# marcinmiklitz/pywindow

Measured on AMD Instinct MI355X. Metric: trajectory frames/sec full_analysis (pore+windows), CC3 1k-frame, higher is better.
Workload: dtype f64

## Files before the change

### pywindow_amd/csrc/pw_team.hpp

```cpp
#pragma once
#include "pw_common.hpp"

namespace pw {

struct HostTeam {
    static constexpr int NWAVES = 1;
    static constexpr int WSIZE = 1;
    static constexpr int SIZE = 1;
    PW_HD static int tid() { return 0; }
    PW_HD static int lane() { return 0; }
    PW_HD static int wave() { return 0; }
    PW_HD static void sync() {}
    PW_HD static void wave_sync() {}
    PW_HD static void wave_argmin(double& v, int& idx) { (void)v; (void)idx; }
    PW_HD static void wave_argmax(double& v, int& idx) { (void)v; (void)idx; }
    PW_HD static void row_argmin4(double v, int idx, double* outv, int* outi) {
        for (int r = 0; r < 4; ++r) { outv[r] = v; outi[r] = idx; }
    }
    PW_HD static double wave_min(double v) { return v; }
    PW_HD static void row_min4(double v, double* outv) { for (int r = 0; r < 4; ++r) outv[r] = v; }
    PW_HD static unsigned long long ballot(bool p) { return p ? 1ull : 0ull; }
    PW_HD static bool wave_all(bool p) { return p; }
    PW_HD static bool wave_any(bool p) { return p; }
    PW_HD static double xor_d(double v, int ) { return v; }
    PW_HD static double bcast(double v, int ) { return v; }
    PW_HD static double bcast_u(double v, int ) { return v; }
    PW_HD static int bcast_i(int v, int ) { return v; }
    PW_HD static int shfl_up_i(int v, int ) { return v; }
    PW_HD static int uniform_i(int v) { return v; }
};

#if defined(__HIPCC__)
#if defined(PW_BARRIER_PROF)
__shared__ unsigned long long pw_bar_acc[8];
#endif
template <int NW>
struct DeviceTeam {
    static constexpr int NWAVES = NW;
    static constexpr int WSIZE = 64;
    static constexpr int SIZE = NW * 64;
    __device__ static int tid() { return threadIdx.x; }
    __device__ static int lane() { return threadIdx.x & 63; }
    __device__ static int wave() { return threadIdx.x >> 6; }
#if defined(PW_BARRIER_PROF)
    __device__ static void sync() {
        const long long t0 = wall_clock64();
        __syncthreads();
        if (lane() == 0) atomicAdd(&pw_bar_acc[wave()], (unsigned long long)(wall_clock64() - t0));
    }
#else
    __device__ static void sync() { __syncthreads(); }
#endif
    __device__ static void wave_sync() {
        __builtin_amdgcn_fence(__ATOMIC_RELEASE, "wavefront");
#if defined(PW_GENERIC_TEAM_MEM)
        asm volatile("s_waitcnt vmcnt(0) lgkmcnt(0)" ::: "memory");
#endif
        __builtin_amdgcn_wave_barrier();
        __builtin_amdgcn_fence(__ATOMIC_ACQUIRE, "wavefront");
    }
    template <int CTRL, int ROW_MASK, int BANK_MASK>
    __device__ static int dpp_i(int x) {
        return __builtin_amdgcn_update_dpp(x, x, CTRL, ROW_MASK, BANK_MASK, false);
    }
    template <int CTRL, int ROW_MASK, int BANK_MASK>
    __device__ static double dpp_d(double x) {
        union { double d; int i[2]; } a, b;
        a.d = x;
        b.i[0] = dpp_i<CTRL, ROW_MASK, BANK_MASK>(a.i[0]);
        b.i[1] = dpp_i<CTRL, ROW_MASK, BANK_MASK>(a.i[1]);
        return b.d;
    }
    __device__ static double lane_d(double x, int lane) {
        union { double d; int i[2]; } a;
        a.d = x;
        a.i[0] = __builtin_amdgcn_readlane(a.i[0], lane);
        a.i[1] = __builtin_amdgcn_readlane(a.i[1], lane);
        return a.d;
    }
    template <bool IS_MIN, int CTRL, int ROW_MASK, int BANK_MASK>
    __device__ static void arg_step(double& v, int& idx) {
        double ov = dpp_d<CTRL, ROW_MASK, BANK_MASK>(v);
        int oi = dpp_i<CTRL, ROW_MASK, BANK_MASK>(idx);
        bool take = IS_MIN ? ((ov < v) || (ov == v && oi < idx)) : ((ov > v) || (ov == v && oi < idx));
        v = take ? ov : v;
        idx = take ? oi : idx;
    }
    template <bool IS_MIN>
    __device__ static void arg_reduce16(double& v, int& idx) {
        arg_step<IS_MIN, 0x111, 0xf, 0xf>(v, idx);
        arg_step<IS_MIN, 0x112, 0xf, 0xf>(v, idx);
        arg_step<IS_MIN, 0x114, 0xf, 0xe>(v, idx);
        arg_step<IS_MIN, 0x118, 0xf, 0xc>(v, idx);
    }
    template <bool IS_MIN>
    __device__ static void arg_reduce64(double& v, int& idx) {
        arg_reduce16<IS_MIN>(v, idx);
        arg_step<IS_MIN, 0x142, 0xa, 0xf>(v, idx);
        arg_step<IS_MIN, 0x143, 0xc, 0xf>(v, idx);
        v = lane_d(v, 63);
        idx = __builtin_amdgcn_readlane(idx, 63);
    }
    __device__ static void wave_argmin(double& v, int& idx) { arg_reduce64<true>(v, idx); }
    __device__ static void wave_argmax(double& v, int& idx) { arg_reduce64<false>(v, idx); }
    __device__ static void row_argmin4(double v, int idx, double* outv, int* outi) {
        arg_reduce16<true>(v, idx);
        outv[0] = lane_d(v, 15); outi[0] = __builtin_amdgcn_readlane(idx, 15);
        outv[1] = lane_d(v, 31); outi[1] = __builtin_amdgcn_readlane(idx, 31);
        outv[2] = lane_d(v, 47); outi[2] = __builtin_amdgcn_readlane(idx, 47);
        outv[3] = lane_d(v, 63); outi[3] = __builtin_amdgcn_readlane(idx, 63);
    }
    template <int CTRL, int ROW_MASK, int BANK_MASK>
    __device__ static void min_step(double& v) {
        v = __builtin_fmin(v, dpp_d<CTRL, ROW_MASK, BANK_MASK>(v));
    }
    __device__ static double wave_min(double v) {
        min_step<0x111, 0xf, 0xf>(v);
        min_step<0x112, 0xf, 0xf>(v);
        min_step<0x114, 0xf, 0xe>(v);
        min_step<0x118, 0xf, 0xc>(v);
        min_step<0x142, 0xa, 0xf>(v);
        min_step<0x143, 0xc, 0xf>(v);
        return lane_d(v, 63);
    }
    __device__ static void row_min4(double v, double* outv) {
        min_step<0x111, 0xf, 0xf>(v);
        min_step<0x112, 0xf, 0xf>(v);
        min_step<0x114, 0xf, 0xe>(v);
        min_step<0x118, 0xf, 0xc>(v);
        outv[0] = lane_d(v, 15); outv[1] = lane_d(v, 31); outv[2] = lane_d(v, 47); outv[3] = lane_d(v, 63);
    }
    __device__ static unsigned long long ballot(bool p) { return __ballot(p); }
    __device__ static bool wave_all(bool p) { return __all(p); }
    __device__ static bool wave_any(bool p) { return __any(p); }
    __device__ static double xor_d(double v, int lane_mask) { return __shfl_xor(v, lane_mask, 64); }
    __device__ static double bcast(double v, int src) { return __shfl(v, src, 64); }
    __device__ static double bcast_u(double v, int src) { return lane_d(v, __builtin_amdgcn_readfirstlane(src)); }
    __device__ static int bcast_i(int v, int src) { return __shfl(v, src, 64); }
    __device__ static int shfl_up_i(int v, int delta) { return __shfl_up(v, delta, 64); }
    __device__ static int uniform_i(int v) { return __builtin_amdgcn_readfirstlane(v); }
    __device__ static int incl_scan_i(int v) {
        v += __builtin_amdgcn_update_dpp(0, v, 0x111, 0xf, 0xf, false);
        v += __builtin_amdgcn_update_dpp(0, v, 0x112, 0xf, 0xf, false);
        v += __builtin_amdgcn_update_dpp(0, v, 0x114, 0xf, 0xf, false);
        v += __builtin_amdgcn_update_dpp(0, v, 0x118, 0xf, 0xf, false);
        const int r0 = __builtin_amdgcn_readlane(v, 15), r1 = __builtin_amdgcn_readlane(v, 31),
                  r2 = __builtin_amdgcn_readlane(v, 47);
        const int row = (threadIdx.x & 63) >> 4;
        return v + (row >= 1 ? r0 : 0) + (row >= 2 ? r1 : 0) + (row >= 3 ? r2 : 0);
    }
};
#endif

}
```

### pywindow_amd/csrc/pw_unit.hpp

```cpp
#pragma once
#include "../../include/pywindow_amd.h"
#include "pw_lbfgsb.hpp"
#include "pw_math.hpp"
#include "pw_team.hpp"
#include <string.h>

#if defined(PW_PROFILE) && defined(__HIPCC__)
__shared__ unsigned long long pw_prof_lds[32];
#define PW_PROF_BASE(ws) ((unsigned long long*)pw_prof_lds)
#endif
#if defined(PW_PROFILE) && defined(__HIP_DEVICE_COMPILE__)
#define PW_T0(var) long long var = wall_clock64()
#if defined(PW_ZPROF) && defined(PW_LB_FINE)
#define PW_T1(ws, slot, var) do { (void)var; } while (0)
#elif defined(PW_BARRIER_PROF)
#define PW_T1(ws, slot, var) do { (void)var; if (T::lane() == 0) { unsigned long long w_ = 0; \
        for (int k_ = 0; k_ < T::NWAVES; ++k_) w_ += atomicExch(&pw_bar_acc[k_], 0ull); \
        atomicAdd(&pw_prof_lds[slot], w_); } } while (0)
#else
#define PW_T1(ws, slot, var) do { if (T::lane() == 0) atomicAdd(&pw_prof_lds[slot], (unsigned long long)(wall_clock64() - var)); } while (0)
#endif
#else
#define PW_T0(var) do {} while (0)
#define PW_T1(ws, slot, var) do {} while (0)
// ... 946 lines not shown
            double along = pw_fma(rz, uz, pw_fma(rx, ux, ry * uy));
            double q = sq3(rx, ry, rz) - along * along;
            double r2 = F.vdw[i] * F.vdw[i];
            if (q >= 0.0 && q <= r2 * (1.0 + 1e-14)) mask |= 1ull << j;
        }
        while (mask) {
            int j = __builtin_ctzll(mask);
            mask &= mask - 1;
            int i = blk + j;
            double rx = F.x[i] - cen[0], ry = F.y[i] - cen[1], rz = F.z[i] - cen[2];
            double along = pw_fma(rz, uz, pw_fma(rx, ux, ry * uy));
            double sq = sq3(rx, ry, rz);
            double perp = pw_sqrt(sq - along * along);
            double radicand = F.vdw[i] * F.vdw[i] - perp * perp;
            if (radicand > 0.0) {
                double half = pw_sqrt(radicand);
                double tin = along - half, tout = along + half;
                double ix = cen[0] + tin * ux, iy = cen[1] + tin * uy, iz = cen[2] + tin * uz;
                double ox = cen[0] + tout * ux, oy = cen[1] + tout * uy, oz = cen[2] + tout * uz;
                double nin = norm3(ix, iy, iz), nout = norm3(ox, oy, oz);
                if (nin < nout) {
                    any = true;
                    if (nout > far) far = nout;
                }
            }
        }
    }
    *farthest = far;
    return any;
}

PW_NOINLINE PW_HD inline bool ray_scan(const Frame& F, int n, const double* cen, double dx, double dy, double dz,
                                       double* farthest) {
    return ray_scan_impl(F, n, cen, dx, dy, dz, farthest);
}

template <int NR, bool FAR>
PW_HD inline __attribute__((always_inline)) void ray_scan_multi_impl(const Frame& F, int n, const double* cen,
                                                                     const double* dx, const double* dy,
                                                                     const double* dz, bool* hit, double* farthest) {
    static_assert(NR == 4, "the merged exact loop below is written for four rays");
    double ux[NR], uy[NR], uz[NR], far[NR];
    bool any[NR];
#pragma unroll
    for (int r = 0; r < NR; ++r) {
        double nrm = norm3(dx[r], dy[r], dz[r]);
        ux[r] = dx[r] / nrm; uy[r] = dy[r] / nrm; uz[r] = dz[r] / nrm;
        far[r] = -1.0;
        any[r] = false;
    }
    const double c0 = cen[0], c1 = cen[1], c2 = cen[2];
    for (int blk = 0; blk < n; blk += 64) {
        unsigned long long mask[NR];
#pragma unroll
        for (int r = 0; r < NR; ++r) mask[r] = 0ull;
        for (int half = 0; half < 64 && blk + half < n; half += 32) {
            unsigned mh[NR];
#pragma unroll
            for (int r = 0; r < NR; ++r) mh[r] = 0u;
            const int base = blk + half;
            const int jend = n - base < 32 ? n - base : 32;
#pragma unroll 2
            for (int j = 0; j < jend; ++j) {
                int i = base + j;
                double rx = F.x[i] - c0, ry = F.y[i] - c1, rz = F.z[i] - c2;
                double rr = sq3(rx, ry, rz);
                double lim = pw_fma(rr, 1e-12, (F.vdw[i] * F.vdw[i]) * (1.0 + 1e-12));
                const unsigned bit = 1u << j;
#pragma unroll
                for (int r = 0; r < NR; ++r) {
                    double along = pw_fma(rz, uz[r], pw_fma(rx, ux[r], ry * uy[r]));
                    double q = pw_fma(-along, along, rr);
                    mh[r] |= q <= lim ? bit : 0u;
                }
            }
#pragma unroll
            for (int r = 0; r < NR; ++r) mask[r] |= (unsigned long long)mh[r] << half;
        }
        if (!FAR) {
#pragma unroll
            for (int r = 0; r < NR; ++r) mask[r] = any[r] ? 0ull : mask[r];
        }
        while ((mask[0] | mask[1] | mask[2] | mask[3]) != 0ull) {
            const int r = mask[0] ? 0 : (mask[1] ? 1 : (mask[2] ? 2 : 3));
            const unsigned long long m = r == 0 ? mask[0] : (r == 1 ? mask[1] : (r == 2 ? mask[2] : mask[3]));
            const unsigned long long rest = m & (m - 1);
            const int i = blk + __builtin_ctzll(m);
            const double vx = r == 0 ? ux[0] : (r == 1 ? ux[1] : (r == 2 ? ux[2] : ux[3]));
            const double vy = r == 0 ? uy[0] : (r == 1 ? uy[1] : (r == 2 ? uy[2] : uy[3]));
            const double vz = r == 0 ? uz[0] : (r == 1 ? uz[1] : (r == 2 ? uz[2] : uz[3]));
            bool got = false;
            double nout = -1.0;
            double rx = F.x[i] - c0, ry = F.y[i] - c1, rz = F.z[i] - c2;
            double along = pw_fma(rz, vz, pw_fma(rx, vx, ry * vy));
            double sq = sq3(rx, ry, rz);
            double perp = pw_sqrt(sq - along * along);
            double radicand = F.vdw[i] * F.vdw[i] - perp * perp;
            if (radicand > 0.0) {
                double half = pw_sqrt(radicand);
                double tin = along - half, tout = along + half;
                double ix = c0 + tin * vx, iy = c1 + tin * vy, iz = c2 + tin * vz;
                double ox = c0 + tout * vx, oy = c1 + tout * vy, oz = c2 + tout * vz;
                double nin = norm3(ix, iy, iz);
                nout = norm3(ox, oy, oz);
                got = nin < nout;
            }
#pragma unroll
            for (int q = 0; q < NR; ++q) {
                const bool mine = r == q;
                if (mine) mask[q] = (!FAR && got) ? 0ull : rest;
                if (mine && got) {
                    any[q] = true;
                    if (FAR && nout > far[q]) far[q] = nout;
                }
            }
        }
    }
#pragma unroll
    for (int r = 0; r < NR; ++r) { hit[r] = any[r]; farthest[r] = far[r]; }
}
template <int NR, bool FAR = true>
PW_NOINLINE PW_HD inline void ray_scan_multi(const Frame& F, int n, const double* cen, const double* dx,
                                             const double* dy, const double* dz, bool* hit, double* farthest) {
    ray_scan_multi_impl<NR, FAR>(F, n, cen, dx, dy, dz, hit, farthest);
}


PW_HD inline void team_store_max_pos(double* p, double v) {
#if defined(__HIP_DEVICE_COMPILE__)
    atomicMax((long long*)p, __double_as_longlong(v));
#else
    if (v > *p) *p = v;
#endif
}
template <class P>
struct SpiralRays {
    P pts;
    int Q4;
    static constexpr int STEP64 = 16;
    PW_HD int first(int k) const { return (k & 3) * Q4 + (k >> 2); }
    PW_HD void at(int off, double* x, double* y, double* z) const { *x = pts[off]; *y = pts[off + 4 * Q4]; *z = pts[off + 8 * Q4]; }
    PW_HD void operator()(int k, double* x, double* y, double* z) const { at(first(k), x, y, z); }
};
template <class P>
struct PlanarRays {
    P a;
    int n;
    static constexpr int STEP64 = 64;
    PW_HD int first(int k) const { return k; }
    PW_HD void at(int off, double* x, double* y, double* z) const { *x = a[off]; *y = a[n + off]; *z = a[2 * n + off]; }
    PW_HD void operator()(int k, double* x, double* y, double* z) const { at(k, x, y, z); }
};
struct ConeBand { double thr; int klo, khi; };
template <class T, bool FAR, class GETP>
PW_HD inline __attribute__((always_inline)) bool team_ray_tests(const Frame& F, int n, const double* cen, const Sphere& sp,
                                                               GETP getp, ConeBand* bands, unsigned* pairs, int cap,
                                                               PW_LDS int* counts, unsigned char* flag,
                                                               unsigned char hit_value, double* far) {
    const int P = sp.P;
    const int seg = cap / T::NWAVES;
    if (P >= 65536 || n >= 65536 || seg < 64) return false;
    const double c0 = cen[0], c1 = cen[1], c2 = cen[2];
    const double cn = norm3(c0, c1, c2);
    for (int i = T::tid(); i < n; i += T::SIZE) {
        const double rx = F.x[i] - c0, ry = F.y[i] - c1, rz = F.z[i] - c2, vr = F.vdw[i];
        const double rr = sq3(rx, ry, rz);
        const double a2 = rr - pw_fma(rr, 1e-12, (vr * vr) * (1.0 + 1e-12));
        ConeBand b;
        b.klo = 0; b.khi = -P;
        b.thr = -PW_INF;
        if (a2 > 0.0) {
            const double amin = pw_sqrt(a2) * (1.0 - 1e-9);
            b.thr = amin * sp.R * (1.0 - 1e-9);
            if (amin > cn + 1e-6) {
                const double len = pw_sqrt(rr);
                const double zd = rz / len, c = amin / len;
                const double s_ = pw_sqrt(pw_max(1.0 - c * c, 0.0)) * (1.0 + 1e-9) + 1e-9;
                const double rho = pw_sqrt(pw_max(1.0 - zd * zd, 0.0));
                const double zhi = zd >= c ? 1.0 : pw_min(1.0, zd * c + rho * s_ + 1e-9);
                const double zlo = zd <= -c ? -1.0 : pw_max(-1.0, zd * c - rho * s_ - 1e-9);
                const double kh = (zlo - sp.start) / sp.step, kl = (zhi - sp.start) / sp.step;
                b.klo = (int)pw_max(kl - 2.0, 0.0);
                b.khi = (int)pw_min(kh + 3.0, (double)(P - 1));
            }
        }
        bands[i] = b;
    }
    T::sync();
    int mine = 0;
    unsigned* my = pairs + (size_t)T::wave() * seg;
    for (int i = T::wave(); i < n; i += T::NWAVES) {
        const ConeBand b = bands[i];
        const bool two_sided = b.khi < 0;
        const int khi = two_sided ? -b.khi - 1 : b.khi;
        const double rx = F.x[i] - c0, ry = F.y[i] - c1, rz = F.z[i] - c2;
        int off = getp.first(b.klo + T::lane());
        for (int kb = b.klo; kb <= khi; kb += T::WSIZE, off += GETP::STEP64) {
            const int k = kb + T::lane();
            bool f = false;
            if (k <= khi) {
                double px, py, pz;
                if (T::WSIZE == 64) getp.at(off, &px, &py, &pz);
                else getp(k, &px, &py, &pz);
                const double dot = pw_fma(pz, rz, pw_fma(px, rx, py * ry));
                f = two_sided ? pw_abs(dot) >= b.thr : dot >= b.thr;
            }
            const unsigned long long bal = T::ballot(f);
            const int pos = mine + __builtin_popcountll(bal & ((1ull << T::lane()) - 1ull));
            if (f && pos < seg) my[pos] = ((unsigned)k << 16) | (unsigned)i;
            mine += __builtin_popcountll(bal);
        }
    }
    if (T::lane() == 0) counts[T::wave()] = mine;
    T::sync();
    int cum[T::NWAVES + 1];
    cum[0] = 0;
    bool fits = true;
#pragma unroll
    for (int w = 0; w < T::NWAVES; ++w) { const int cw = counts[w]; fits = fits && cw <= seg; cum[w + 1] = cum[w] + cw; }
    T::sync();
    if (!fits) return false;
    for (int g = T::tid(); g < cum[T::NWAVES]; g += T::SIZE) {
        int w = 0, first = 0;
#pragma unroll
        for (int q = 1; q < T::NWAVES; ++q)
            if (g >= cum[q]) { w = q; first = cum[q]; }
        const unsigned pr = pairs[(size_t)w * seg + (g - first)];
        const int k = (int)(pr >> 16), i = (int)(pr & 0xffffu);
        double dx, dy, dz;
        getp(k, &dx, &dy, &dz);
        const double nrm = norm3(dx, dy, dz);
        const double ux = dx / nrm, uy = dy / nrm, uz = dz / nrm;
        const double rx = F.x[i] - c0, ry = F.y[i] - c1, rz = F.z[i] - c2;
        const double along = pw_fma(rz, uz, pw_fma(rx, ux, ry * uy));
        const double sq = sq3(rx, ry, rz);
        const double perp = pw_sqrt(sq - along * along);
        const double radicand = F.vdw[i] * F.vdw[i] - perp * perp;
        if (radicand > 0.0) {
            const double half = pw_sqrt(radicand);
            const double tin = along - half, tout = along + half;
            const double ix = c0 + tin * ux, iy = c1 + tin * uy, iz = c2 + tin * uz;
            const double ox = c0 + tout * ux, oy = c1 + tout * uy, oz = c2 + tout * uz;
            const double nin = norm3(ix, iy, iz), nout = norm3(ox, oy, oz);
            if (nin < nout) {
                flag[k] = hit_value;
                if (FAR) team_store_max_pos(&far[k], nout);
            }
        }
    }
    T::sync();
    return true;
}

PW_HD inline double np_floordiv(double a, double b) {
    double mod = __builtin_fmod(a, b);
    double div = (a - mod) / b;
    if (mod != 0.0) {
        if ((b < 0.0) != (mod < 0.0)) div -= 1.0;
    }
    double fl;
    if (div != 0.0) {
        fl = __builtin_floor(div);
        if (div - fl > 0.5) fl += 1.0;
    } else {
        fl = 0.0;
    }
    return fl;
}

PW_NOINLINE PW_HD inline bool path_scan_thread(const Frame& F, int n, double vx, double vy, double vz,
                                   double inc, double m0, double* out_2gap, int* out_pos, double* out_chunk,
                                   int* n_eval, const lint* cand = nullptr, const lint* coff = nullptr) {
    double nrm = norm3(vx, vy, vz);
    int chunks = (int)np_floordiv(nrm, inc);
    double cx = vx / (double)chunks, cy = vy / (double)chunks, cz = vz / (double)chunks;
    double best = PW_INF;
    int pos = 0;
    bool ok = true;
    int k0 = 0;
    if (chunks >= 1) {
        if (!(m0 > 0.0)) ok = false;
        best = m0;
        k0 = 1;
    }
    auto tile = [&](auto np_) __attribute__((always_inline)) {
        constexpr int NP = decltype(np_)::value;
        double qx[NP], qy[NP], qz[NP], m[NP];
#pragma unroll
        for (int p = 0; p < NP; ++p) {
            int k = k0 + p <= chunks ? k0 + p : chunks;
            qx[p] = cx * (double)k; qy[p] = cy * (double)k; qz[p] = cz * (double)k;
        }
        points_gap_values<NP>(F, n, qx, qy, qz, m, cand, coff);
#pragma unroll
        for (int p = 0; p < NP; ++p) {
            if (k0 + p <= chunks && ok) {
                if (!(m[p] > 0.0)) ok = false;
                else if (m[p] < best) { best = m[p]; pos = k0 + p; }
            }
        }
        k0 += NP;
    };
    while (k0 <= chunks && ok) {
        if (chunks - k0 + 1 <= 5) tile(std::integral_constant<int, 5>());
        else tile(std::integral_constant<int, 6>());
    }
    if (n_eval) *n_eval += chunks + 1;
    if (!ok) return false;
    *out_2gap = best * 2.0;
    *out_pos = pos;
    out_chunk[0] = cx; out_chunk[1] = cy; out_chunk[2] = cz;
    return true;
}

template <class T>
PW_HD inline bool wave_path_candidates(const Frame& F, int n, bool have, double vx, double vy, double vz, double inc,
                                       double m0, lint* cand, lint* coff) {
    const auto& C = *F.cls;
    if (C.k == 0 || !(m0 > 0.0)) return false;
    double uz_lo = PW_INF, uz_hi = -PW_INF, t1 = PW_INF;
    bool odd = false;
    if (have) {
        const double nrm = norm3(vx, vy, vz);
        odd = !(nrm >= inc * (1.0 + 1e-9)) || !(nrm < PW_INF) || !(inc > 0.0);
        if (!odd) uz_lo = uz_hi = vz / nrm;
    }
    if (T::wave_any(odd)) return false;
    double z1 = T::wave_min(uz_lo) - 1e-9, z2 = -T::wave_min(-uz_hi) + 1e-9;
    t1 = inc * (1.0 - 1e-9);
    if (!(z1 <= z2)) return false;
    z1 = pw_max(z1, -1.0); z2 = pw_min(z2, 1.0);
    const double s1 = pw_sqrt(pw_max(1.0 - z1 * z1, 0.0)), s2 = pw_sqrt(pw_max(1.0 - z2 * z2, 0.0));
    const double m0p = m0 * (1.0 + 1e-9) + 1e-9;
    const int mycut = T::lane() <= C.k ? C.off[T::lane() <= PW_KCLS ? T::lane() : PW_KCLS] : n;
    int mycount = 0, cnt = 0;
    for (int base = 0; base < n; base += T::WSIZE) {
        const int i = base + T::lane();
        bool keep = false;
        if (i < n) {
            const double xx = F.xx[i], z = F.z[i], r = F.vdw[i];
            const double rho = pw_sqrt(xx);
            const double zd = rho > 0.0 ? z / rho : 0.0;
            const double sd = pw_sqrt(pw_max(1.0 - zd * zd, 0.0));
            double c1 = 1.0;
            if (zd > z2) c1 = sd * s2 + zd * z2;
// ... 689 lines not shown
#endif
            LB_F0(f_post);
            double f0 = -(gv[0] * 2.0);
            for (int c = 0; c < 3; ++c) {
                double f1 = -(gv[c + 1] * 2.0);
                lg[c] = (f1 - f0) / dxs[c];
            }
            lf = f0;
            lx = px; ly = py; lz = pz;
            have_last = true;
            nfev += 4;
            LB_F1(28, f_post);
        }
        fo = lf;
        go[0] = lg[0]; go[1] = lg[1]; go[2] = lg[2];
    }
};

template <class T>
PW_HD inline __attribute__((always_inline)) void stage_opt_impl(UnitShared& sh, TeamWorkspace* ws, int n, pw_unit_out* out,
                                                                const pw_params& prm) {
    (void)ws;
    auto& v = *sh.v;
    if (T::wave() == 0) {
        const Frame A = sh.A;
        Lbfgsb<3> opt;
        Lbfgsb<3>* S = &opt;
        LbMem<3>* Smem = (LbMem<3>*)sh.lb[0];
        PW_ASSUME_LDS(Smem);
        double r = v.pore_g;
        double lo[3], up[3], x0[3];
        int nbd[3] = {2, 2, 2};
        for (int c = 0; c < 3; ++c) x0[c] = (prm.opt_flags & PW_OPT_CUSTOM_START) ? prm.opt_x0[c] : v.com[c];
        if ((prm.opt_flags & PW_OPT_CUSTOM_START) && !(prm.opt_flags & PW_OPT_CUSTOM_BOUNDS))
            r = wave_gap<T>(A, n, x0[0], x0[1], x0[2], nullptr);
        bool bad;
        if (prm.opt_flags & PW_OPT_CUSTOM_BOUNDS) {
            bad = false;
            for (int c = 0; c < 3; ++c) {
                lo[c] = prm.opt_lo[c];
                up[c] = prm.opt_hi[c];
                bool has_lo = lo[c] > -PW_INF, has_up = up[c] < PW_INF;
                nbd[c] = has_lo ? (has_up ? 2 : 1) : (has_up ? 3 : 0);
                if (lo[c] > up[c]) bad = true;
                x0[c] = x0[c] < lo[c] ? lo[c] : (x0[c] > up[c] ? up[c] : x0[c]);
            }
        } else {
            for (int c = 0; c < 3; ++c) {
                lo[c] = x0[c] - r;
                up[c] = x0[c] + r;
            }
            bad = !(r > 0.0);
        }
        int nit = 0, nfev = 0;
        if (!bad) {
            S->template setup<T>(Smem, x0, lo, up, nbd, 1e7, 1e-5, 20);
#if defined(PW_PROFILE) && !defined(PW_ZPROF)
            S->prof = PW_PROF_BASE(ws);
#endif
#if defined(PW_PROFILE) && defined(PW_LB_FINE) && !defined(PW_ZPROF)
            Smem->prof_fine = PW_PROF_BASE(ws);
#endif
            PoreObjective<T> fg(A, n, lo, up, (PW_LDS int*)Smem->cand);
#if defined(PW_PROFILE) && !defined(PW_ZPROF)
            fg.prof = PW_PROF_BASE(ws);
#endif
            PW_T0(t_s);
            S->template minimize<T>(fg, 15000, 15000, &nit);
            T::wave_sync();
            PW_T1(ws, 0, t_s);
            nfev = fg.nfev;
        }
        double cx = v.com[0], cy = v.com[1], cz = v.com[2];
        if (!bad) { cx = S->x[0]; cy = S->x[1]; cz = S->x[2]; }
        int arg;
        double g = wave_gap<T>(A, n, cx, cy, cz, &arg);
        if (T::lane() == 0) {
            v.opt_c[0] = cx; v.opt_c[1] = cy; v.opt_c[2] = cz;
            v.opt_g = g;
            v.opt_atom = arg;
            v.n_eval += nfev + 1;
            if (bad) v.status |= PW_ST_NEGATIVE_PORE;
            out->pore_opt_d = g * 2.0;
            out->pore_opt_atom = arg;
            out->pore_opt_c[0] = cx; out->pore_opt_c[1] = cy; out->pore_opt_c[2] = cz;
            double rr = out->pore_opt_d / 2.0;
            out->pore_vol_opt = FOUR_THIRDS_PI * pw_cube_np(rr);
            out->opt_nit = nit;
            out->opt_nfev = nfev;
            out->opt_task = bad ? -1 : S->task;
            out->opt_msg = bad ? 0 : S->msg;
        }
    }
    T::sync();
}

template <class T>
PW_NOINLINE PW_HD inline void stage_opt(UnitShared& sh, TeamWorkspace* ws, int n, pw_unit_out* out,
                                        const pw_params& prm) {
    stage_opt_impl<T>(sh, ws, n, out, prm);
}

template <class T>
PW_NOINLINE PW_HD inline void stage_average(UnitShared& sh, TeamWorkspace* ws, int n, pw_unit_out* out,
                                             const pw_params& prm) {
    auto& v = *sh.v;
    PW_T0(t_a0);
    make_shifted<T>(sh, n, v.com[0], v.com[1], v.com[2]);
    double keep_d = v.maxd;
    int keep_i = v.maxd_i, keep_j = v.maxd_j;
    T::sync();
    {
        double* ib = 2 * n + 2 <= ws->p_cap ? ws->vals : nullptr;
        team_max_dim<T, true>(sh, sh.S, n, ib);
    }
    double radius = v.maxd;
    T::sync();
    if (T::tid() == 0) { v.maxd = keep_d; v.maxd_i = keep_i; v.maxd_j = keep_j; }
    int P = sampling_count(radius, prm.adjust_average);
    if (P > ws->p_cap) {
        if (T::tid() == 0) { v.status |= PW_ST_POINTS_OVERFLOW; out->avg_d = __builtin_nan(""); out->n_points_avg = P; }
        T::sync();
        return;
    }
    Sphere sp;
    sp.init(radius, P);
    ScratchArena arena;
    arena.init(sh);
    double* vals = (double*)arena.take((size_t)P * 8);
    if (!vals) vals = ws->vals;
    double* packed = vals;
    unsigned char* flag = (unsigned char*)arena.take((size_t)P);
    if (!flag) flag = ws->flag;
    int* s_tab = (int*)arena.take(324 * 4);
    size_t acc_words = 8 * (size_t)(((P < 8192 ? P : 8192) + 63) / 64);
    if (acc_words < 128) acc_words = 128;
    double* s_acc = (double*)arena.take(acc_words * 8);
    double* s_leaf = (double*)arena.take(256 * 8);
    if (!s_tab || !s_acc || !s_leaf) { s_tab = ws->leaf_tab; s_acc = ws->acc8; s_leaf = ws->leaf; }
    double cen[3] = {v.centroid[0], v.centroid[1], v.centroid[2]};
    if (T::wave() == 0) PW_T1(ws, 27, t_a0);
    PW_T0(t_a1);
    bool done = false;
    {
        ScratchArena a2 = arena;
        double* apts = (double*)a2.take((size_t)P * 24);
        if (apts) {
            team_sphere_points<T>(ws, sp, [&](int k, double x, double y, double z) {
                apts[k] = x; apts[P + k] = y; apts[2 * P + k] = z;
                vals[k] = -1.0;
                flag[k] = 0;
            });
            ConeBand* bands = (ConeBand*)a2.take((size_t)n * sizeof(ConeBand));
            int cap = (int)(a2.left / 4);
            unsigned* pairs = (unsigned*)a2.take((size_t)cap * 4);
            if (cap < 4 * P) { pairs = (unsigned*)ws->knn; cap = 16 * ws->p_cap; }
            if (!bands && (size_t)n * sizeof(ConeBand) <= (size_t)ws->p_cap * 16) bands = (ConeBand*)(ws->knn + 8 * (size_t)ws->p_cap);
            PlanarRays<decltype(PW_AS_LDS(apts))> getp{PW_AS_LDS(apts), P};
            if (bands)
                done = team_ray_tests<T, true>(sh.S, n, cen, sp, getp, bands, pairs, cap, (PW_LDS int*)&v.red_i[0], flag, 1, vals);
        }
    }
    if (done) {
    } else if (T::SIZE > 1) {
        constexpr int NR = 4;
        for (int k0 = T::tid(); k0 < P; k0 += NR * T::SIZE) {
            double dx[NR], dy[NR], dz[NR], far[NR];
            bool hit[NR];
#pragma unroll
            for (int r = 0; r < NR; ++r) {
                int k = k0 + r * T::SIZE < P ? k0 + r * T::SIZE : k0;
                sp.point(k, &dx[r], &dy[r], &dz[r]);
            }
            ray_scan_multi<NR>(sh.S, n, cen, dx, dy, dz, hit, far);
#pragma unroll
            for (int r = 0; r < NR; ++r) {
                int k = k0 + r * T::SIZE;
                if (k < P) { vals[k] = far[r]; flag[k] = hit[r] ? 1 : 0; }
            }
        }
    } else {
        for (int k = T::tid(); k < P; k += T::SIZE) {
            double px, py, pz, far;
            sp.point(k, &px, &py, &pz);
            bool hit = ray_scan(sh.S, n, cen, px, py, pz, &far);
            vals[k] = far;
            flag[k] = hit ? 1 : 0;
        }
    }
    T::sync();
    if (T::wave() == 0) PW_T1(ws, 28, t_a1);
    PW_T0(t_a2);
    if (T::wave() == 0) {
        int m = 0;
        for (int base = 0; base < P; base += T::WSIZE) {
            int k = base + T::lane();
            bool f = k < P && flag[k] != 0;
            unsigned long long bal = T::ballot(f);
            int pos = m + __builtin_popcountll(bal & ((1ull << T::lane()) - 1ull));
            if (f) packed[pos] = vals[k];
            m += __builtin_popcountll(bal);
        }
        if (T::lane() == 0) v.n_surv = m;
    }
    T::sync();
    int m = v.n_surv;
    double sum = np_sum_team<T>(packed, m, s_tab, s_acc, s_leaf, &v.red_v[15]);
    if (T::wave() == 0) PW_T1(ws, 29, t_a2);
    if (T::tid() == 0) {
        out->avg_d = (sum / (double)m) * 2.0;
        out->n_points_avg = P;
    }
    T::sync();
}

template <class T>
PW_NOINLINE PW_HD inline void wave_fmin_xy(const Frame& F, int n, double z, double x0, double y0, double* xo,
                               double* yo, int* n_eval) {
    const int maxfun = 400, maxiter = 400;
    const double xatol = 1e-4, fatol = 1e-4;
    double x0s, y0s, f0s, x1s, y1s, f1s, x2s, y2s, f2s;
    int fcalls = 0;
#if defined(__HIP_DEVICE_COMPILE__)
    NearGap1<T> near_gap;
    near_gap.init();
    const Frame Fl = F;
    auto fun = [&](double x, double y) {
        fcalls += 1;
        if (T::WSIZE == 64) return -(near_gap.eval(Fl, n, nullptr, x, y, z) * 2.0);
        return -(wave_gap_value<T>(Fl, n, x, y, z) * 2.0);
    };
#else
    auto fun = [&](double x, double y) {
        fcalls += 1;
        return -(wave_gap_value<T>(F, n, x, y, z) * 2.0);
    };
#endif
    x0s = x0; y0s = y0;
    x1s = (x0 != 0.0) ? (1.0 + 0.05) * x0 : 0.00025; y1s = y0;
    x2s = x0; y2s = (y0 != 0.0) ? (1.0 + 0.05) * y0 : 0.00025;
    f0s = fun(x0s, y0s);
    f1s = fun(x1s, y1s);
    f2s = fun(x2s, y2s);
    auto swap01 = [&]() { double t; t = f0s; f0s = f1s; f1s = t; t = x0s; x0s = x1s; x1s = t; t = y0s; y0s = y1s; y1s = t; };
    auto swap12 = [&]() { double t; t = f1s; f1s = f2s; f2s = t; t = x1s; x1s = x2s; x2s = t; t = y1s; y1s = y2s; y2s = t; };
    auto sort3 = [&]() {
        if (f0s > f1s) swap01();
        if (f1s > f2s) { swap12(); if (f0s > f1s) swap01(); }
    };
    sort3();
    int iterations = 1;
    while (fcalls < maxfun && iterations < maxiter) {
        double dx1 = pw_abs(x1s - x0s), dx2 = pw_abs(x2s - x0s);
        double dy1 = pw_abs(y1s - y0s), dy2 = pw_abs(y2s - y0s);
        double mx = pw_max(pw_max(dx1, dy1), pw_max(dx2, dy2));
        double mf = pw_max(pw_abs(f0s - f1s), pw_abs(f0s - f2s));
        if (mx <= xatol && mf <= fatol) break;
        double bx = (x0s + x1s) / 2.0, by = (y0s + y1s) / 2.0;
        double xr = 2.0 * bx - x2s, yr = 2.0 * by - y2s;
        bool over = false;
        auto guarded = [&](double x, double y, double* f) {
            if (fcalls >= maxfun) { over = true; return false; }
            *f = fun(x, y);
            return true;
        };
        double fxr;
        if (guarded(xr, yr, &fxr)) {
            bool doshrink = false;
            if (fxr < f0s) {
                double xe = 3.0 * bx - 2.0 * x2s, ye = 3.0 * by - 2.0 * y2s;
                double fxe;
                if (guarded(xe, ye, &fxe)) {
                    if (fxe < fxr) { x2s = xe; y2s = ye; f2s = fxe; }
                    else { x2s = xr; y2s = yr; f2s = fxr; }
                }
            } else if (fxr < f1s) {
                x2s = xr; y2s = yr; f2s = fxr;
            } else if (fxr < f2s) {
                double xc = 1.5 * bx - 0.5 * x2s, yc = 1.5 * by - 0.5 * y2s;
                double fxc;
                if (guarded(xc, yc, &fxc)) {
                    if (fxc <= fxr) { x2s = xc; y2s = yc; f2s = fxc; }
                    else doshrink = true;
                }
            } else {
                double xcc = 0.5 * bx + 0.5 * x2s, ycc = 0.5 * by + 0.5 * y2s;
                double fxcc;
                if (guarded(xcc, ycc, &fxcc)) {
                    if (fxcc < f2s) { x2s = xcc; y2s = ycc; f2s = fxcc; }
                    else doshrink = true;
                }
            }
            if (doshrink && !over) {
                x1s = x0s + 0.5 * (x1s - x0s);
                y1s = y0s + 0.5 * (y1s - y0s);
                double f;
                if (guarded(x1s, y1s, &f)) f1s = f;
                if (!over) {
                    x2s = x0s + 0.5 * (x2s - x0s);
                    y2s = y0s + 0.5 * (y2s - y0s);
                    if (guarded(x2s, y2s, &f)) f2s = f;
                }
            }
            if (!over) iterations += 1;
        }
        sort3();
    }
    *xo = x0s;
    *yo = y0s;
    *n_eval += fcalls;
}

template <class T>
// ... 855 lines not shown
#pragma unroll
            for (int c = 0; c < PW_NB_K; ++c) {
                const int j = (int)((w[c >> 1] >> (16 * (c & 1))) & 0xffffu);
                const double qx = pts_[PT(j, 0)], qy = pts_[PT(j, 1)], qz = pts_[PT(j, 2)];
                double ax = px - qx, ay = py - qy, az = pz - qz;
                double d = ax * ax;
                d = d + ay * ay; d = d + az * az;
                sorted = sorted && d >= prev;
                prev = d;
                cd[c] = d;
                if (c < 10) d10[c] = d;
            }
            if (!sorted) {
#pragma unroll
                for (int q = 0; q < 10; ++q) d10[q] = PW_INF;
#pragma unroll
                for (int c = 0; c < PW_NB_K; ++c) {
                    double v_ = cd[c];
#pragma unroll
                    for (int q = 0; q < 10; ++q) {
                        double lo_ = __builtin_fmin(d10[q], v_);
                        v_ = __builtin_fmax(d10[q], v_);
                        d10[q] = lo_;
                    }
                }
            }
            const bool ok = d10[9] < nb_bound[k] * slack;
#pragma unroll
            for (int q = 0; q < 10; ++q) d10[q] = pw_sqrt(d10[q]);
            return ok;
        };
        auto point_dists = [&](auto pts_, int grp, int k, bool& searched, double* d10) __attribute__((always_inline)) {
            if (!searched && point_tabled(pts_, k, d10)) return;
            if (!searched) {
                knn_window_group(pts_, Q4, P, grp, W, radius, zstep, ws->knn);
                searched = true;
            }
#pragma unroll
            for (int q = 0; q < 10; ++q) d10[q] = ws->knn[(size_t)k * 10 + q];
        };
        if (!streamed) {
            auto rows_of_groups = [&](auto pts_) __attribute__((always_inline)) {
                for (int grp = T::tid(); grp < ngroups; grp += T::SIZE) {
                    bool searched = false;
                    for (int p = 0; p < NK; ++p) {
                        const int k = grp * NK + p;
                        if (k >= P) break;
                        double d10[10];
                        point_dists(pts_, grp, k, searched, d10);
                        if (!searched) {
#pragma unroll
                            for (int q = 0; q < 10; ++q) ws->knn[(size_t)k * 10 + q] = d10[q];
                        }
                    }
                }
            };
            if (PW_IS_LDS(pts)) rows_of_groups(PW_AS_LDS(pts)); else rows_of_groups(pts);
        }
        T::sync();
        if (T::wave() == 0) PW_T1(ws, 24, t_knn);
        PW_T0(t_sum);
        double sum;
        if (streamed) {
            const int n_el = P * 10;
            const int grp = T::tid();
            const int e_first = grp * NK * 10;
            bool searched = false;
            double total = 0.0;
            bool first = true;
            for (int s0 = 0; s0 < n_el; s0 += 8192) {
                const int len = n_el - s0 < 8192 ? n_el - s0 : 8192;
                np_leaf_table<T>(len, s_tab);
                int lo = 0;
                while (lo < len) {
                    int hi = len;
                    if (lo + tile_cap < len) {
                        int off, l;
                        np_descend(len, lo + tile_cap, &off, &l);
                        hi = off;
                    }
                    auto fill = [&](auto tile_, auto pts_) __attribute__((always_inline)) {
                        if (nb_idx) {
                            const int E0 = s0 + lo, E1 = s0 + hi;
                            const int k1 = (E1 - 1) / 10;
                            for (int k = E0 / 10 + T::tid(); k <= k1; k += T::SIZE) {
                                double d10[10];
                                if (!point_tabled(pts_, k, d10)) {
                                    knn_window_group(pts_, Q4, P, k / NK, W, radius, zstep, ws->knn);
#pragma unroll
                                    for (int q = 0; q < 10; ++q) d10[q] = ws->knn[(size_t)k * 10 + q];
                                }
                                const int e0 = k * 10 - s0;
#pragma unroll
                                for (int q = 0; q < 10; ++q)
                                    if (e0 + q >= lo && e0 + q < hi) tile_[e0 + q - lo] = d10[q];
                            }
                            return;
                        }
                        if (grp >= ngroups) return;
                        for (int p = 0; p < NK; ++p) {
                            const int k = grp * NK + p;
                            const int e0 = e_first + p * 10 - s0;
                            if (k >= P || e0 + 10 <= lo || e0 >= hi) continue;
                            double d10[10];
                            point_dists(pts_, grp, k, searched, d10);
#pragma unroll
                            for (int q = 0; q < 10; ++q)
                                if (e0 + q >= lo && e0 + q < hi) tile_[e0 + q - lo] = d10[q];
                        }
                    };
                    if (PW_IS_LDS(tile) && PW_IS_LDS(pts)) fill(PW_AS_LDS(tile), PW_AS_LDS(pts)); else fill(tile, pts);
                    T::sync();
                    np_leaf_phase<T>(tile, len, lo, hi, s_tab, s_acc, s_leaf, true);
                    lo = hi;
                }
                double part = np_walk_phase<T>(len, s_tab, s_acc, s_leaf);
                if (T::tid() == 0) total = first ? part : total + part;
                first = false;
                T::sync();
            }
            if (T::tid() == 0) v.red_v[15] = total;
            T::sync();
            sum = v.red_v[15];
            T::sync();
        } else {
            sum = np_sum_team<T>(ws->knn, P * 10, s_tab, s_acc, s_leaf, &v.red_v[15]);
        }
        double m = sum / (double)(P * 10);
        if (T::tid() == 0) { v.eps = m + pw_pow_np(m, 0.5); out->eps = v.eps; }
        T::sync();
        if (T::wave() == 0) PW_T1(ws, 25, t_sum);
    }
    if (T::wave() == 0) PW_T1(ws, 8, t_eps);
    PW_T0(t_smp);
    arena = arena_pts;
    double* vals = (double*)arena.take((size_t)P * 8);
    if (!vals) vals = ws->vals;
    int* surv_k = (int*)arena.take((size_t)P * 4);
    if (!surv_k) surv_k = ws->surv_k;
    int* labels = (int*)arena.take((size_t)P * 4);
    if (!labels) labels = ws->labels;
    unsigned char* flag = (unsigned char*)arena.take((size_t)P);
    if (!flag) flag = ws->flag;
    ScratchArena arena_mark = arena;
    double* tmpv = (double*)arena.take((size_t)P * 8);
    if (!tmpv) tmpv = ws->knn;
    {
        double cen[3] = {v.centroid[0], v.centroid[1], v.centroid[2]};
        bool done = false;
        {
            for (int k = T::tid(); k < P; k += T::SIZE) flag[k] = 1;
            ScratchArena a2 = arena_mark;
            ConeBand* bands = (ConeBand*)a2.take((size_t)n * sizeof(ConeBand));
            int cap = (int)(a2.left / 4);
            unsigned* pairs = (unsigned*)a2.take((size_t)cap * 4);
            if (cap < 4 * P) { pairs = (unsigned*)ws->knn; cap = 16 * ws->p_cap; }
            if (!bands && (size_t)n * sizeof(ConeBand) <= (size_t)ws->p_cap * 16) bands = (ConeBand*)(ws->knn + 8 * (size_t)ws->p_cap);
            auto run = [&](auto pts_) __attribute__((always_inline)) {
                SpiralRays<decltype(pts_)> getp{pts_, Q4};
                return team_ray_tests<T, false>(sh.S, n, cen, sp, getp, bands, pairs, cap, (PW_LDS int*)&v.red_i[0], flag, 0, nullptr);
            };
            if (bands) done = PW_IS_LDS(pts) ? run(PW_AS_LDS(pts)) : run(pts);
        }
        if (done) {
        } else if (T::SIZE > 1) {
            constexpr int NR = 4;
            for (int k0 = T::tid(); k0 < P; k0 += NR * T::SIZE) {
                double dx[NR], dy[NR], dz[NR], far[NR];
                bool hit[NR];
#pragma unroll
                for (int r = 0; r < NR; ++r) {
                    int k = k0 + r * T::SIZE < P ? k0 + r * T::SIZE : k0;
                    dx[r] = pts[PT(k, 0)]; dy[r] = pts[PT(k, 1)]; dz[r] = pts[PT(k, 2)];
                }
                ray_scan_multi<NR, false>(sh.S, n, cen, dx, dy, dz, hit, far);
#pragma unroll
                for (int r = 0; r < NR; ++r) {
                    int k = k0 + r * T::SIZE;
                    if (k < P) flag[k] = hit[r] ? 0 : 1;
                }
            }
        } else {
            for (int k = T::tid(); k < P; k += T::SIZE) {
                double far;
                bool hit = ray_scan(sh.S, n, cen, pts[PT(k, 0)], pts[PT(k, 1)], pts[PT(k, 2)], &far);
                flag[k] = hit ? 0 : 1;
            }
        }
        T::sync();
        if (T::wave() == 0) {
            int m = 0;
            for (int base = 0; base < P; base += T::WSIZE) {
                int k = base + T::lane();
                bool f = k < P && flag[k] != 0;
                unsigned long long bal = T::ballot(f);
                int pos = m + __builtin_popcountll(bal & ((1ull << T::lane()) - 1ull));
                if (f) labels[pos] = k;
                m += __builtin_popcountll(bal);
            }
            if (T::lane() == 0) v.n_surv = m;
        }
        T::sync();
        int ncand = v.n_surv;
        int evals = 0;
        if (T::wave() == 0) PW_T1(ws, 30, t_smp);
        PW_T0(t_path);
        const double m_origin = wave_gap_value<T>(sh.S, n, 0.0, 0.0, 0.0);
        int whole = T::SIZE > 1 ? (ncand / T::SIZE) * T::SIZE : ncand;
        if ((ncand - whole) * 16 >= T::SIZE) whole = ncand;
        lint* cand_w = nullptr;
        lint* coff_w = nullptr;
        {
            ScratchArena a3 = arena;
            const size_t per_wave = (size_t)n + PW_KCLS + 2;
            int* c_all = (int*)a3.take((size_t)T::NWAVES * per_wave * 4);
#ifndef PW_NO_SCAN_LISTS
            if (c_all && PW_IS_LDS(c_all)) {
                cand_w = (lint*)PW_AS_LDS(c_all) + (size_t)T::wave() * per_wave;
                coff_w = cand_w + n;
            }
#endif
        }
        for (int j0 = 0; j0 < whole; j0 += T::SIZE) {
            const int j = j0 + T::tid();
            const bool have = j < whole;
            const int k = have ? labels[j] : 0;
            const double vx = pts[PT(k, 0)], vy = pts[PT(k, 1)], vz = pts[PT(k, 2)];
            const bool listed = cand_w != nullptr &&
                                wave_path_candidates<T>(sh.S, n, have, vx, vy, vz, prm.increment, m_origin, cand_w, coff_w);
            if (have) {
                double g2, chunk[3];
                int pos;
                bool ok = path_scan_thread(sh.S, n, vx, vy, vz, prm.increment, m_origin, &g2, &pos, chunk, &evals,
                                           listed ? cand_w : nullptr, listed ? coff_w : nullptr);
                flag[j] = ok ? 1 : 0;
                tmpv[j] = g2;
            }
        }
        const int left = ncand - whole;
        if (left > 0) {
            for (int j = whole + T::wave(); j < ncand; j += T::NWAVES) {
                const int k = labels[j];
                const double vx = pts[PT(k, 0)], vy = pts[PT(k, 1)], vz = pts[PT(k, 2)];
                const int chunks = (int)np_floordiv(norm3(vx, vy, vz), prm.increment);
                double g2 = 0.0;
                bool ok = true;
                bool all_at_once = false;
                if constexpr (T::WSIZE == 64) all_at_once = chunks >= 1 && chunks <= 16 && sh.S.cls->k > 0;
                if (all_at_once) {
                    if constexpr (T::WSIZE == 64) {
                        const auto& C = *sh.S.cls;
                        const Frame& F = sh.S;
                        const double cx = vx / (double)chunks, cy = vy / (double)chunks, cz = vz / (double)chunks;
                        const int sub = T::lane() & 3;
                        const int q = (T::lane() >> 2) + 1 <= chunks ? (T::lane() >> 2) + 1 : chunks;
                        const double qx = cx * (double)q, qy = cy * (double)q, qz = cz * (double)q;
                        const double pp = sq3(qx, qy, qz);
                        double gap = PW_INF;
                        for (int g = 0; g < C.k; ++g) {
                            double m2 = PW_INF;
                            const int hi = C.off[g + 1];
                            for (int i = C.off[g] + sub; i < hi; i += 4) {
                                const double x = F.x[i], y = F.y[i], z = F.z[i], xx = F.xx[i];
                                const double gg = pw_fma(z, qz, pw_fma(x, qx, y * qy));
                                m2 = __builtin_fmin(m2, pw_m2add(gg, xx));
                            }
                            m2 = __builtin_fmin(m2, T::xor_d(m2, 1));
                            m2 = __builtin_fmin(m2, T::xor_d(m2, 2));
                            const double m2p = m2 + pp;
                            const double d = pw_sqrt(m2p > 0.0 ? m2p : 0.0);
                            gap = __builtin_fmin(gap, d - C.vdw[g]);
                        }
                        double best = m_origin;
                        if (!(m_origin > 0.0)) ok = false;
                        for (int q2 = 1; q2 <= chunks && ok; ++q2) {
                            const double m = T::bcast_u(gap, 4 * (q2 - 1));
                            if (!(m > 0.0)) ok = false;
                            else if (m < best) best = m;
                        }
                        g2 = best * 2.0;
                    }
                } else if (chunks >= 1) {
                    const double cx = vx / (double)chunks, cy = vy / (double)chunks, cz = vz / (double)chunks;
                    double best = m_origin;
                    if (!(m_origin > 0.0)) ok = false;
                    for (int q = 1; q <= chunks && ok; ++q) {
                        const double m = wave_gap_value<T>(sh.S, n, cx * (double)q, cy * (double)q, cz * (double)q);
                        if (!(m > 0.0)) ok = false;
                        else if (m < best) best = m;
                    }
                    g2 = best * 2.0;
                } else {
                    double chunk[3];
                    int pos;
                    ok = path_scan_thread(sh.S, n, vx, vy, vz, prm.increment, m_origin, &g2, &pos, chunk, &evals);
                }
                if (T::lane() == 0) { flag[j] = ok ? 1 : 0; tmpv[j] = g2; }
            }
        }
        T::sync();
        if (T::wave() == 0) PW_T1(ws, 31, t_path);
        if (T::wave() == 0) {
            int m = 0;
            for (int base = 0; base < ncand; base += T::WSIZE) {
                int j = base + T::lane();
                bool f = j < ncand && flag[j] != 0;
                unsigned long long bal = T::ballot(f);
                int pos = m + __builtin_popcountll(bal & ((1ull << T::lane()) - 1ull));
                if (f) { surv_k[pos] = labels[j]; vals[pos] = tmpv[j]; }
                m += __builtin_popcountll(bal);
            }
            if (T::lane() == 0) { v.n_surv = m; out->n_survivors = m; }
        }
// ... 207 lines not shown
```

Measured before the change: 976,600.

## Enumerate cone-ray candidates via golden-angle lattice walk instead of band scans

```diff
diff --git a/pywindow_amd/csrc/pw_team.hpp b/pywindow_amd/csrc/pw_team.hpp
--- a/pywindow_amd/csrc/pw_team.hpp
+++ b/pywindow_amd/csrc/pw_team.hpp
@@ -28,6 +28,7 @@
     PW_HD static int bcast_i(int v, int ) { return v; }
     PW_HD static int shfl_up_i(int v, int ) { return v; }
     PW_HD static int uniform_i(int v) { return v; }
+    PW_HD static int incl_scan_i(int v) { return v; }
 };
 
 #if defined(__HIPCC__)
diff --git a/pywindow_amd/csrc/pw_unit.hpp b/pywindow_amd/csrc/pw_unit.hpp
--- a/pywindow_amd/csrc/pw_unit.hpp
+++ b/pywindow_amd/csrc/pw_unit.hpp
@@ -1122,45 +1122,222 @@
     PW_HD void operator()(int k, double* x, double* y, double* z) const { at(k, x, y, z); }
 };
 struct ConeBand { double thr; int klo, khi; };
+
+struct ConeLatticeTable {
+    static constexpr int N = 25;
+    int q[N];
+    double s[N];
+    constexpr ConeLatticeTable() : q{}, s{} {
+        int a = 1, b = 2;
+        for (int i = 0; i < N; ++i) {
+            const double x = (double)a * (GOLDEN_ANGLE / TWO_PI);
+            q[i] = a;
+            s[i] = x - (double)(long)(x + 0.5);
+            const int c = a + b; a = b; b = c;
+        }
+    }
+};
+constexpr ConeLatticeTable CONE_LATTICE_TABLE{};
+constexpr double CONE_LATTICE_G = GOLDEN_ANGLE / TWO_PI;
+#ifndef PW_CONE_TARGET
+#define PW_CONE_TARGET 12
+#endif
+constexpr double CONE_TARGET = PW_CONE_TARGET;
+struct ConeLattice { double c, w; int first; short j; unsigned short plen; };
+PW_HD inline int cone_pieces(int band, double w, unsigned short* plen) {
+    if (band <= 0) { *plen = 1; return 0; }
+    int want = (int)((double)band * w / CONE_TARGET) + 1;
+    if (want > band) want = band;
+    const int len = (band + want - 1) / want;
+    *plen = (unsigned short)len;
+    return (band + len - 1) / len;
+}
+PW_HD inline double cone_asin(double x) {
+#if defined(__HIP_DEVICE_COMPILE__)
+    return ::asin(x);
+#else
+    return __builtin_asin(x);
+#endif
+}
+PW_HD inline double cone_atan2(double y, double x) {
+#if defined(__HIP_DEVICE_COMPILE__)
+    return ::atan2(y, x);
+#else
+    return __builtin_atan2(y, x);
+#endif
+}
+PW_HD inline ConeLattice cone_lattice_window(double rx, double ry, double rz, double rr, double thr, double R) {
+    ConeLattice L;
+    L.c = 0.0; L.w = 1.0; L.j = -1; L.first = 0; L.plen = 1;
+    const double len = pw_sqrt(rr);
+    const double ct = thr / (R * len) - 1e-12;
+    if (!(ct > 0.0)) return L;
+    const double sa = pw_sqrt(pw_max(1.0 - ct * ct, 0.0));
+    const double rho = pw_sqrt(rx * rx + ry * ry) / len;
+    if (!(rho > sa * (1.0 + 1e-6) + 1e-9)) return L;
+    const double delta = cone_asin(sa / rho) * (1.0 + 1e-9) + 1e-9;
+    const double w = delta / ONE_PI;
+    int j = 0;
+    while (j + 1 < ConeLatticeTable::N && pw_abs(CONE_LATTICE_TABLE.s[j]) > w) ++j;
+    if (j + 1 >= ConeLatticeTable::N) return L;
+    double c = (cone_atan2(ry, rx) - delta) / TWO_PI;
+    c -= __builtin_floor(c);
+    L.c = c < 1.0 ? c : 0.0;
+    L.w = w;
+    L.j = (short)j;
+    return L;
+}
+struct ConeLatticeWalk {
+    double t, w, a, b;
+    int k, A, B;
+    PW_HD void enter(const ConeLattice& L, int k0, int kend) {
+        const int j = L.j, pos = j & 1 ? j + 1 : j, neg = j & 1 ? j : j + 1;
+        A = CONE_LATTICE_TABLE.q[pos]; a = CONE_LATTICE_TABLE.s[pos];
+        B = CONE_LATTICE_TABLE.q[neg]; b = -CONE_LATTICE_TABLE.s[neg];
+        w = L.w;
+        k = k0;
+        t = (double)k0 * CONE_LATTICE_G - L.c;
+        t -= __builtin_floor(t);
+        while (k <= kend && !(t < w)) {
+            ++k;
+            t += CONE_LATTICE_G;
+            if (t >= 1.0) t -= 1.0;
+        }
+    }
+    PW_HD void next() {
+        if (t + a < w) { k += A; t += a; }
+        else if (t - b >= 0.0) { k += B; t -= b; }
+        else { k += A + B; t = (t + a) - b; }
+    }
+};
+PW_HD inline ConeLattice* take_cone_lattice(ScratchArena& a, int n) {
+#ifdef PW_NO_CONE_LATTICE
+    (void)a; (void)n;
+    return nullptr;
+#else
+    return (ConeLattice*)a.take((size_t)(n + 1) * sizeof(ConeLattice));
+#endif
+}
+PW_HD inline __attribute__((always_inline)) int cone_of_atom(double rx, double ry, double rz, double vr, double cn, const Sphere& sp,
+                                                            bool narrow, ConeBand* out, ConeLattice* lat_out) {
+    const int P = sp.P;
+    ConeBand b;
+    ConeLattice L;
+    L.c = 0.0; L.w = 1.0; L.j = -1; L.first = 0; L.plen = 1;
+    int cnt = 0;
+    const double rr = sq3(rx, ry, rz);
+    const double a2 = rr - pw_fma(rr, 1e-12, (vr * vr) * (1.0 + 1e-12));
+    b.klo = 0; b.khi = -P;
+    b.thr = -PW_INF;
+    if (a2 > 0.0) {
+        const double amin = pw_sqrt(a2) * (1.0 - 1e-9);
+        b.thr = amin * sp.R * (1.0 - 1e-9);
+        if (amin > cn + 1e-6) {
+            const double len = pw_sqrt(rr);
+            const double zd = rz / len, c = amin / len;
+            const double s_ = pw_sqrt(pw_max(1.0 - c * c, 0.0)) * (1.0 + 1e-9) + 1e-9;
+            const double rho = pw_sqrt(pw_max(1.0 - zd * zd, 0.0));
+            const double zhi = zd >= c ? 1.0 : pw_min(1.0, zd * c + rho * s_ + 1e-9);
+            const double zlo = zd <= -c ? -1.0 : pw_max(-1.0, zd * c - rho * s_ - 1e-9);
+            const double kh = (zlo - sp.start) / sp.step, kl = (zhi - sp.start) / sp.step;
+            b.klo = (int)pw_max(kl - 2.0, 0.0);
+            b.khi = (int)pw_min(kh + 3.0, (double)(P - 1));
+            if (narrow) {
+                L = cone_lattice_window(rx, ry, rz, rr, b.thr, sp.R);
+                if (L.j >= 0) {
+                    cnt = cone_pieces(b.khi - b.klo + 1, L.w, &L.plen);
+                    b.klo = ~b.klo;
+                }
+            }
+        }
+    }
+    *out = b;
+    *lat_out = L;
+    return cnt;
+}
 template <class T, bool FAR, class GETP>
 PW_HD inline __attribute__((always_inline)) bool team_ray_tests(const Frame& F, int n, const double* cen, const Sphere& sp,
                                                                GETP getp, ConeBand* bands, unsigned* pairs, int cap,
                                                                PW_LDS int* counts, unsigned char* flag,
-                                                               unsigned char hit_value, double* far) {
+                                                               unsigned char hit_value, double* far,
+                                                               ConeLattice* lat = nullptr) {
     const int P = sp.P;
     const int seg = cap / T::NWAVES;
     if (P >= 65536 || n >= 65536 || seg < 64) return false;
     const double c0 = cen[0], c1 = cen[1], c2 = cen[2];
     const double cn = norm3(c0, c1, c2);
-    for (int i = T::tid(); i < n; i += T::SIZE) {
-        const double rx = F.x[i] - c0, ry = F.y[i] - c1, rz = F.z[i] - c2, vr = F.vdw[i];
-        const double rr = sq3(rx, ry, rz);
-        const double a2 = rr - pw_fma(rr, 1e-12, (vr * vr) * (1.0 + 1e-12));
+    int running = 0;
+    for (int base = 0; base < n; base += T::SIZE) {
+        const int i = base + T::tid();
         ConeBand b;
-        b.klo = 0; b.khi = -P;
-        b.thr = -PW_INF;
-        if (a2 > 0.0) {
-            const double amin = pw_sqrt(a2) * (1.0 - 1e-9);
-            b.thr = amin * sp.R * (1.0 - 1e-9);
-            if (amin > cn + 1e-6) {
-                const double len = pw_sqrt(rr);
-                const double zd = rz / len, c = amin / len;
-                const double s_ = pw_sqrt(pw_max(1.0 - c * c, 0.0)) * (1.0 + 1e-9) + 1e-9;
-                const double rho = pw_sqrt(pw_max(1.0 - zd * zd, 0.0));
-                const double zhi = zd >= c ? 1.0 : pw_min(1.0, zd * c + rho * s_ + 1e-9);
-                const double zlo = zd <= -c ? -1.0 : pw_max(-1.0, zd * c - rho * s_ - 1e-9);
-                const double kh = (zlo - sp.start) / sp.step, kl = (zhi - sp.start) / sp.step;
-                b.klo = (int)pw_max(kl - 2.0, 0.0);
-                b.khi = (int)pw_min(kh + 3.0, (double)(P - 1));
-            }
-        }
-        bands[i] = b;
-    }
+        ConeLattice L;
+        int cnt = 0;
+        if (i < n) {
+            cnt = cone_of_atom(F.x[i] - c0, F.y[i] - c1, F.z[i] - c2, F.vdw[i], cn, sp, lat != nullptr, &b, &L);
+            bands[i] = b;
+        }
+        if (lat != nullptr) {
+            const int inc = T::incl_scan_i(cnt);
+            if (T::lane() == T::WSIZE - 1) counts[T::wave()] = inc;
+            T::sync();
+            int at = running + inc - cnt;
+#pragma unroll
+            for (int w = 0; w < T::NWAVES; ++w) { const int cw = counts[w]; if (w < T::wave()) at += cw; running += cw; }
+            if (i < n) { L.first = at; lat[i] = L; }
+            T::sync();
+        }
+    }
+    if (lat != nullptr && T::tid() == 0) lat[n].first = running;
     T::sync();
     int mine = 0;
     unsigned* my = pairs + (size_t)T::wave() * seg;
+    auto enumerate = [&](auto bands_, auto lat_, auto my_) __attribute__((always_inline)) {
+        for (int g0 = T::wave() * T::WSIZE; g0 < running; g0 += T::SIZE) {
+            const int g = g0 + T::lane();
+            ConeLatticeWalk wk;
+            wk.k = 1;
+            int kend = 0, i = 0;
+            double rx = 0.0, ry = 0.0, rz = 0.0, thr = 0.0;
+            if (g < running) {
+                int lo = 0, hi = n - 1;
+                while (lo < hi) {
+                    const int mid = (lo + hi) >> 1;
+                    if (lat_[mid + 1].first > g) hi = mid; else lo = mid + 1;
+                }
+                i = lo;
+                const ConeBand b = bands_[i];
+                const ConeLattice L = lat_[i];
+                const int k0 = ~b.klo + (g - L.first) * (int)L.plen;
+                kend = k0 + (int)L.plen - 1 < b.khi ? k0 + (int)L.plen - 1 : b.khi;
+                rx = F.x[i] - c0; ry = F.y[i] - c1; rz = F.z[i] - c2;
+                thr = b.thr;
+                wk.enter(L, k0, kend);
+            }
+            while (T::wave_any(wk.k <= kend)) {
+                const bool act = wk.k <= kend;
+                const int k = wk.k;
+                bool f = false;
+                if (act) {
+                    double px, py, pz;
+                    getp(k, &px, &py, &pz);
+                    const double dot = pw_fma(pz, rz, pw_fma(px, rx, py * ry));
+                    f = dot >= thr;
+                    wk.next();
+                }
+                const unsigned long long bal = T::ballot(f);
+                const int pos = mine + __builtin_popcountll(bal & ((1ull << T::lane()) - 1ull));
+                if (f && pos < seg) my_[pos] = ((unsigned)k << 16) | (unsigned)i;
+                mine += __builtin_popcountll(bal);
+            }
+        }
+    };
+    if (lat != nullptr) {
+        if (PW_IS_LDS(bands) && PW_IS_LDS(lat) && PW_IS_LDS(my)) enumerate(PW_AS_LDS(bands), PW_AS_LDS(lat), PW_AS_LDS(my));
+        else enumerate(bands, lat, my);
+    }
     for (int i = T::wave(); i < n; i += T::NWAVES) {
         const ConeBand b = bands[i];
+        if (b.klo < 0) continue;
         const bool two_sided = b.khi < 0;
         const int khi = two_sided ? -b.khi - 1 : b.khi;
         const double rx = F.x[i] - c0, ry = F.y[i] - c1, rz = F.z[i] - c2;
@@ -2156,13 +2333,14 @@
                 flag[k] = 0;
             });
             ConeBand* bands = (ConeBand*)a2.take((size_t)n * sizeof(ConeBand));
+            ConeLattice* lat = bands ? take_cone_lattice(a2, n) : nullptr;
             int cap = (int)(a2.left / 4);
             unsigned* pairs = (unsigned*)a2.take((size_t)cap * 4);
             if (cap < 4 * P) { pairs = (unsigned*)ws->knn; cap = 16 * ws->p_cap; }
             if (!bands && (size_t)n * sizeof(ConeBand) <= (size_t)ws->p_cap * 16) bands = (ConeBand*)(ws->knn + 8 * (size_t)ws->p_cap);
             PlanarRays<decltype(PW_AS_LDS(apts))> getp{PW_AS_LDS(apts), P};
             if (bands)
-                done = team_ray_tests<T, true>(sh.S, n, cen, sp, getp, bands, pairs, cap, (PW_LDS int*)&v.red_i[0], flag, 1, vals);
+                done = team_ray_tests<T, true>(sh.S, n, cen, sp, getp, bands, pairs, cap, (PW_LDS int*)&v.red_i[0], flag, 1, vals, lat);
         }
     }
     if (done) {
@@ -3324,13 +3502,14 @@
             for (int k = T::tid(); k < P; k += T::SIZE) flag[k] = 1;
             ScratchArena a2 = arena_mark;
             ConeBand* bands = (ConeBand*)a2.take((size_t)n * sizeof(ConeBand));
+            ConeLattice* lat = bands ? take_cone_lattice(a2, n) : nullptr;
             int cap = (int)(a2.left / 4);
             unsigned* pairs = (unsigned*)a2.take((size_t)cap * 4);
             if (cap < 4 * P) { pairs = (unsigned*)ws->knn; cap = 16 * ws->p_cap; }
             if (!bands && (size_t)n * sizeof(ConeBand) <= (size_t)ws->p_cap * 16) bands = (ConeBand*)(ws->knn + 8 * (size_t)ws->p_cap);
             auto run = [&](auto pts_) __attribute__((always_inline)) {
                 SpiralRays<decltype(pts_)> getp{pts_, Q4};
-                return team_ray_tests<T, false>(sh.S, n, cen, sp, getp, bands, pairs, cap, (PW_LDS int*)&v.red_i[0], flag, 0, nullptr);
+                return team_ray_tests<T, false>(sh.S, n, cen, sp, getp, bands, pairs, cap, (PW_LDS int*)&v.red_i[0], flag, 0, nullptr, lat);
             };
             if (bands) done = PW_IS_LDS(pts) ? run(PW_AS_LDS(pts)) : run(pts);
         }
```

Measured after the change: 1.010 million, median of 6. 1.03x the previous value.
